# jackroos/VL-BERT

Measured on AMD Instinct MI355X. Metric: samples/sec VL-BERT-base pretrain (seq 64+36 regions) at 1/2/4/8 MI355X, higher is better.
Workload: dtype bf16; 1 GPU; VL-BERT-base 12-layer pretrain step (fwd+bwd+clip+AdamW), 64 text + 36 regions, precomputed 2048-d region features, dropout on; global_batch=256, per_gpu_batch=256, per_gpu_caption_samples=256, per_gpu_text_only_samples=0, module=ResNetVLBERTForPretraining, seq_len=101, parallelism=dp1, hipgraph=False, arch=gfx950:sramecc+:xnack-, cus=256, forced_exchange=False, ranks=1

## Files before the change

### vl-bert_amd/csrc/attention.hip

```cpp
#include "vlb_common.h"

#define ATT_SP_MAX 256
#define ATT_D 64
#define ATT_THREADS 512

typedef __attribute__((ext_vector_type(4))) short s16x4;
typedef __attribute__((ext_vector_type(8))) short s16x8;

__device__ __forceinline__ int rho(int s) { return (s & ~31) | (((s >> 2) & 1) << 4) | (((s >> 3) & 3) << 2) | (s & 3); }
__device__ __forceinline__ int rm_addr(int row, int chunk) { return row * 128 + ((chunk ^ ((row >> 1) & 7)) << 4); }
__device__ __forceinline__ bf16x8 lds_frag(const char* base, int addr) { return *(const bf16x8*)(base + addr); }

__device__ __forceinline__ bf16x8 frag_perm(const char* img, int blk, int half, int c, int chunk) {
  return lds_frag(img, rm_addr(32 * blk + 16 * half + c, chunk));
}
__device__ __forceinline__ bf16x8 frag_nat(const char* img, int s0, int c, int chunk) {
  return lds_frag(img, rm_addr(rho(s0 + c), chunk));
}
__device__ __forceinline__ bf16x8 frag_tr(const char* img, int blk, int d0, int lane) {
  const int L = lane & 15, g = lane >> 4;
  const int b = d0 * 2 + (L & 3) * 8;
  const int r_lo = 32 * blk + 4 * g + (L >> 2);
  const int r_hi = r_lo + 16;
  const int a_lo = r_lo * 128 + ((((b >> 4) ^ ((r_lo >> 1) & 7)) << 4) | (b & 15));
  const int a_hi = r_hi * 128 + ((((b >> 4) ^ ((r_hi >> 1) & 7)) << 4) | (b & 15));
  const s16x4 lo = __builtin_amdgcn_ds_read_tr16_b64_v4i16((__attribute__((address_space(3))) s16x4*)(img + a_lo));
  const s16x4 hi = __builtin_amdgcn_ds_read_tr16_b64_v4i16((__attribute__((address_space(3))) s16x4*)(img + a_hi));
  const s16x8 v = __builtin_shufflevector(lo, hi, 0, 1, 2, 3, 4, 5, 6, 7);
  return __builtin_bit_cast(bf16x8, v);
}

template <int SP>
struct TileRegs {
  uint4 v[SP * 8 / ATT_THREADS];
};

template <int SP>
__device__ __forceinline__ void tile_load(const bf16_t* __restrict__ g, long ld, int S, int tid, TileRegs<SP>& r) {
#pragma unroll
  for (int it = 0; it < SP * 8 / ATT_THREADS; ++it) {
    const int P = it * ATT_THREADS + tid, s = min(P >> 3, S - 1), ch = P & 7;
    r.v[it] = *(const uint4*)(g + (long)s * ld + ch * 8);
  }
}

template <int SP>
__device__ __forceinline__ void tile_store(const TileRegs<SP>& r, int S, char* img, int tid) {
#pragma unroll
  for (int it = 0; it < SP * 8 / ATT_THREADS; ++it) {
    const int P = it * ATT_THREADS + tid, s = P >> 3, ch = P & 7;
    const bool in = s < S;
    const uint4 v = make_uint4(in ? r.v[it].x : 0u, in ? r.v[it].y : 0u, in ? r.v[it].z : 0u, in ? r.v[it].w : 0u);
    *(uint4*)(img + rm_addr(rho(s), ch)) = v;
  }
}

template <int SP>
__device__ __forceinline__ void rowdot_store(const TileRegs<SP>& a_, const TileRegs<SP>& o_, int S, float* sD, int tid) {
#pragma unroll
  for (int it = 0; it < SP * 8 / ATT_THREADS; ++it) {
    const int P = it * ATT_THREADS + tid, row = P >> 3, ch = P & 7;
    const uint4 a = a_.v[it], o = o_.v[it];
    float d = bflo(a.x) * bflo(o.x) + bfhi(a.x) * bfhi(o.x) + bflo(a.y) * bflo(o.y) + bfhi(a.y) * bfhi(o.y) +
              bflo(a.z) * bflo(o.z) + bfhi(a.z) * bfhi(o.z) + bflo(a.w) * bflo(o.w) + bfhi(a.w) * bfhi(o.w);
    d = row < S ? d : 0.f;
    d += __shfl_xor(d, 1, 64);
    d += __shfl_xor(d, 2, 64);
    d += __shfl_xor(d, 4, 64);
    if (ch == 0) sD[row] = d;
  }
}

__device__ __forceinline__ bf16x8 pack8(const float* v) {
  uint32_t w[4] = {pack2bf(v[0], v[1]), pack2bf(v[2], v[3]), pack2bf(v[4], v[5]), pack2bf(v[6], v[7])};
  return __builtin_bit_cast(bf16x8, *(uint4*)w);
}

__device__ __forceinline__ void drop8(float* v, uint32_t key, uint32_t base, uint32_t thr, float scale) {
  const uint32_t odd = base & 1u, p0 = base >> 1;
  uint32_t h[5];
#pragma unroll
  for (int k = 0; k < 5; ++k) h[k] = vlb_pair_hash(p0 + k, key);
#pragma unroll
  for (int k = 0; k < 4; ++k) {
    const uint32_t w = __builtin_amdgcn_alignbit(h[k + 1], h[k], odd << 4);
    v[2 * k] = ((w & 0xffffu) >= thr) ? v[2 * k] * scale : 0.f;
    v[2 * k + 1] = ((w >> 16) >= thr) ? v[2 * k + 1] * scale : 0.f;
  }
}

struct AttnParams {
  const bf16_t* qkv;
  const float* mask;
  bf16_t* ctx;
  float* lse;
  const bf16_t* dctx;
  bf16_t* dqkv;
  int B, S, H, nh;
  float scale;
  uint32_t drop_thr; float drop_scale; const uint32_t* seed; uint32_t tag;
};

template <int NU, int QS>
__global__ __launch_bounds__(ATT_THREADS, NU <= 4 ? 4 : 2) void attn_fwd_kernel(const AttnParams p) {
  constexpr int ATT_SP = 32 * NU, TILE_BYTES = ATT_SP * ATT_D * 2;
  extern __shared__ __attribute__((aligned(16))) char smem[];
  char* sK = smem;
  char* sV = smem + TILE_BYTES;
  float* sMB = (float*)(smem + 2 * TILE_BYTES);

  const int tid = threadIdx.x, lane = tid & 63, wave = tid >> 6;
  const int c = lane & 15, g = lane >> 4;
  const int b = blockIdx.x / p.nh, h = blockIdx.x % p.nh;
  const int S = p.S;
  const long ld = 3L * p.H;
  const bf16_t* qbase = p.qkv + (long)b * S * ld + h * ATT_D;
  TileRegs<ATT_SP> rk, rv;
  tile_load<ATT_SP>(qbase + p.H, ld, S, tid, rk);
  tile_load<ATT_SP>(qbase + 2 * p.H, ld, S, tid, rv);
  bf16x8 qf[2];
  auto load_q = [&](int q0) {
    const int q = min(q0 + c, S - 1);
#pragma unroll
    for (int ds = 0; ds < 2; ++ds) qf[ds] = *(const bf16x8*)(qbase + (long)q * ld + ds * 32 + g * 8);
  };
  load_q(wave * 16);
  const float mrow = p.mask[b * S + min(tid, S - 1)];
  const uint32_t seed = (p.drop_thr && p.seed) ? *p.seed : 0u;
  tile_store<ATT_SP>(rk, S, sK, tid);
  tile_store<ATT_SP>(rv, S, sV, tid);
  if (tid < ATT_SP) sMB[tid] = (tid < S) ? (1.0f - mrow) * -10000.0f : -INFINITY;
  __syncthreads();
  const uint32_t key = vlb_rng_key(seed, p.tag);
  const int U = (S + 31) >> 5;

#pragma unroll 1
  for (int qs = 0; qs < QS; ++qs) {
  const int q0 = (wave + 8 * qs) * 16;
  if (q0 >= S) break;
  if (qs > 0) load_q(q0);

  f32x4 sc[NU][2];
#pragma unroll
  for (int u = 0; u < NU; ++u)
#pragma unroll
    for (int hf = 0; hf < 2; ++hf) {
      sc[u][hf] = (f32x4){0.f, 0.f, 0.f, 0.f};
      if (u < U) {
#pragma unroll
        for (int ds = 0; ds < 2; ++ds)
          sc[u][hf] = VLB_MFMA_16x16x32(frag_perm(sK, u, hf, c, ds * 4 + g), qf[ds], sc[u][hf], 0, 0, 0);
      }
    }

  float mx = -INFINITY;
#pragma unroll
  for (int u = 0; u < NU; ++u)
#pragma unroll
    for (int hf = 0; hf < 2; ++hf)
#pragma unroll
      for (int r = 0; r < 4; ++r) {
        const float v = (u < U) ? sc[u][hf][r] * p.scale + sMB[32 * u + 8 * g + 4 * hf + r] : -INFINITY;
        sc[u][hf][r] = v;
        mx = fmaxf(mx, v);
      }
  mx = fmaxf(mx, __shfl_xor(mx, 16, 64));
  mx = fmaxf(mx, __shfl_xor(mx, 32, 64));
  float sum = 0.f;
#pragma unroll
  for (int u = 0; u < NU; ++u)
#pragma unroll
    for (int hf = 0; hf < 2; ++hf)
#pragma unroll
      for (int r = 0; r < 4; ++r) {
        const float e = __expf(sc[u][hf][r] - mx);
        sc[u][hf][r] = e;
        sum += e;
      }
  sum += __shfl_xor(sum, 16, 64);
  sum += __shfl_xor(sum, 32, 64);
  const float inv = 1.0f / sum;
  const int q = q0 + c;
  if (g == 0 && q < S) p.lse[((long)b * p.nh + h) * S + q] = mx + __logf(sum);

  const uint32_t qrow = ((uint32_t)(b * p.nh + h) * (uint32_t)S + (uint32_t)min(q, S - 1)) * (uint32_t)S;
  bf16x8 pf[NU];
#pragma unroll
  for (int u = 0; u < NU; ++u) {
    float v[8];
#pragma unroll
    for (int hf = 0; hf < 2; ++hf)
#pragma unroll
      for (int r = 0; r < 4; ++r) v[4 * hf + r] = sc[u][hf][r] * inv;
    if (p.drop_thr) drop8(v, key, qrow + 32u * u + 8u * g, p.drop_thr, p.drop_scale);
    pf[u] = pack8(v);
  }

  bf16_t* orow = p.ctx + ((long)b * S + min(q, S - 1)) * p.H + h * ATT_D + 4 * g;
#pragma unroll
  for (int dt = 0; dt < 4; ++dt) {
    f32x4 o = {0.f, 0.f, 0.f, 0.f};
#pragma unroll
    for (int u = 0; u < NU; ++u)
      if (u < U) o = VLB_MFMA_16x16x32(frag_tr(sV, u, dt * 16, lane), pf[u], o, 0, 0, 0);
    if (q < S) *(uint2*)(orow + dt * 16) = make_uint2(pack2bf(o[0], o[1]), pack2bf(o[2], o[3]));
  }
  }
}

template <int NU, int QS>
__global__ __launch_bounds__(ATT_THREADS, NU <= 4 ? 4 : 2) void attn_bwd_kernel(const AttnParams p) {
  constexpr int ATT_SP = 32 * NU, TILE_BYTES = ATT_SP * ATT_D * 2;
  extern __shared__ __attribute__((aligned(16))) char smem[];
  char* sQ = smem;
  char* sK = smem + 1 * TILE_BYTES;
  char* sV = smem + 2 * TILE_BYTES;
  char* sdO = smem + 3 * TILE_BYTES;
  float* sMB = (float*)(smem + 4 * TILE_BYTES);
  float* sLSE = sMB + ATT_SP;
  float* sD = sLSE + ATT_SP;

  const int tid = threadIdx.x, lane = tid & 63, wave = tid >> 6;
  const int c = lane & 15, g = lane >> 4;
  const int b = blockIdx.x / p.nh, h = blockIdx.x % p.nh;
  const int S = p.S;
  const long ld = 3L * p.H;
  const bf16_t* qbase = p.qkv + (long)b * S * ld + h * ATT_D;
  const bf16_t* dobase = p.dctx + (long)b * S * p.H + h * ATT_D;
  const bf16_t* obase = p.ctx + (long)b * S * p.H + h * ATT_D;
  TileRegs<ATT_SP> rq, rk, rv, rdo, ro;
  tile_load<ATT_SP>(qbase, ld, S, tid, rq);
  tile_load<ATT_SP>(qbase + p.H, ld, S, tid, rk);
  tile_load<ATT_SP>(qbase + 2 * p.H, ld, S, tid, rv);
  tile_load<ATT_SP>(dobase, p.H, S, tid, rdo);
  tile_load<ATT_SP>(obase, p.H, S, tid, ro);
  const float mrow = p.mask[b * S + min(tid, S - 1)];
  const float lrow = p.lse[((long)b * p.nh + h) * S + min(tid, S - 1)];
  const uint32_t seed = (p.drop_thr && p.seed) ? *p.seed : 0u;
  tile_store<ATT_SP>(rq, S, sQ, tid);
  tile_store<ATT_SP>(rk, S, sK, tid);
  tile_store<ATT_SP>(rv, S, sV, tid);
  tile_store<ATT_SP>(rdo, S, sdO, tid);
  rowdot_store<ATT_SP>(rdo, ro, S, sD, tid);
  if (tid < ATT_SP) {
    sMB[tid] = (tid < S) ? (1.0f - mrow) * -10000.0f : -INFINITY;
    sLSE[tid] = (tid < S) ? lrow : 0.f;
  }
  __syncthreads();

  const uint32_t key = vlb_rng_key(seed, p.tag);
  const uint32_t bh = (uint32_t)(b * p.nh + h);
  const int U = (S + 31) >> 5;
#pragma unroll 1
  for (int qs = 0; qs < QS; ++qs) {
  const int w16 = (wave + 8 * qs) * 16;
  if (w16 >= S) break;
  const int pos = w16 + c;
  const bool pos_ok = pos < S;

  {
    bf16x8 kf[2], vf[2];
#pragma unroll
    for (int ds = 0; ds < 2; ++ds) {
      kf[ds] = frag_nat(sK, w16, c, ds * 4 + g);
      vf[ds] = frag_nat(sV, w16, c, ds * 4 + g);
    }
    f32x4 dv[4], dk[4];
#pragma unroll
    for (int dt = 0; dt < 4; ++dt) dv[dt] = dk[dt] = (f32x4){0.f, 0.f, 0.f, 0.f};
    const float mb = sMB[pos];
    const uint32_t kcol = (uint32_t)min(pos, S - 1);
#pragma unroll (NU <= 4 ? NU : 1)
    for (int v = 0; v < NU; ++v) {
      if (v < U) {
        float pv[8], dsv[8];
#pragma unroll
        for (int hf = 0; hf < 2; ++hf) {
          f32x4 s = {0.f, 0.f, 0.f, 0.f}, dp = {0.f, 0.f, 0.f, 0.f};
#pragma unroll
          for (int ds = 0; ds < 2; ++ds) {
            s = VLB_MFMA_16x16x32(frag_perm(sQ, v, hf, c, ds * 4 + g), kf[ds], s, 0, 0, 0);
            dp = VLB_MFMA_16x16x32(frag_perm(sdO, v, hf, c, ds * 4 + g), vf[ds], dp, 0, 0, 0);
          }
#pragma unroll
          for (int r = 0; r < 4; ++r) {
            const int q = 32 * v + 8 * g + 4 * hf + r;
            const float pr = __expf(s[r] * p.scale + mb - sLSE[q]);
            float keepf = 1.f;
            if (p.drop_thr) {
              const uint32_t idx = (bh * (uint32_t)S + (uint32_t)min(q, S - 1)) * (uint32_t)S + kcol;
              const uint32_t hsh = vlb_pair_hash(idx >> 1, key);
              keepf = (((idx & 1u) ? (hsh >> 16) : (hsh & 0xffffu)) >= p.drop_thr) ? p.drop_scale : 0.f;
            }
            pv[4 * hf + r] = pr * keepf;
            dsv[4 * hf + r] = pr * (dp[r] * keepf - sD[q]);
          }
        }
        const bf16x8 pd = pack8(pv), dsf = pack8(dsv);
#pragma unroll
        for (int dt = 0; dt < 4; ++dt) {
          dv[dt] = VLB_MFMA_16x16x32(frag_tr(sdO, v, dt * 16, lane), pd, dv[dt], 0, 0, 0);
          dk[dt] = VLB_MFMA_16x16x32(frag_tr(sQ, v, dt * 16, lane), dsf, dk[dt], 0, 0, 0);
        }
      }
    }
    if (pos_ok) {
      bf16_t* orow = p.dqkv + ((long)b * S + pos) * ld + h * ATT_D + 4 * g;
#pragma unroll
      for (int dt = 0; dt < 4; ++dt) {
        *(uint2*)(orow + p.H + dt * 16) = make_uint2(pack2bf(dk[dt][0] * p.scale, dk[dt][1] * p.scale),
                                                     pack2bf(dk[dt][2] * p.scale, dk[dt][3] * p.scale));
        *(uint2*)(orow + 2 * p.H + dt * 16) = make_uint2(pack2bf(dv[dt][0], dv[dt][1]), pack2bf(dv[dt][2], dv[dt][3]));
      }
    }
  }

  {
    bf16x8 qf[2], dof[2];
#pragma unroll
    for (int ds = 0; ds < 2; ++ds) {
      qf[ds] = frag_nat(sQ, w16, c, ds * 4 + g);
      dof[ds] = frag_nat(sdO, w16, c, ds * 4 + g);
    }
    f32x4 dq[4];
#pragma unroll
    for (int dt = 0; dt < 4; ++dt) dq[dt] = (f32x4){0.f, 0.f, 0.f, 0.f};
    const float lse = sLSE[pos], dd = sD[pos];
    const uint32_t qrow = (bh * (uint32_t)S + (uint32_t)min(pos, S - 1)) * (uint32_t)S;
#pragma unroll (NU <= 4 ? NU : 1)
    for (int u = 0; u < NU; ++u) {
      if (u < U) {
        float pr[8], dpv[8];
#pragma unroll
        for (int hf = 0; hf < 2; ++hf) {
          f32x4 s = {0.f, 0.f, 0.f, 0.f}, dp = {0.f, 0.f, 0.f, 0.f};
#pragma unroll
          for (int ds = 0; ds < 2; ++ds) {
            s = VLB_MFMA_16x16x32(frag_perm(sK, u, hf, c, ds * 4 + g), qf[ds], s, 0, 0, 0);
            dp = VLB_MFMA_16x16x32(frag_perm(sV, u, hf, c, ds * 4 + g), dof[ds], dp, 0, 0, 0);
          }
#pragma unroll
          for (int r = 0; r < 4; ++r) {
            pr[4 * hf + r] = __expf(s[r] * p.scale + sMB[32 * u + 8 * g + 4 * hf + r] - lse);
            dpv[4 * hf + r] = dp[r];
          }
        }
        if (p.drop_thr) drop8(dpv, key, qrow + 32u * u + 8u * g, p.drop_thr, p.drop_scale);
        float dsv[8];
#pragma unroll
        for (int j = 0; j < 8; ++j) dsv[j] = pr[j] * (dpv[j] - dd);
        const bf16x8 dsf = pack8(dsv);
#pragma unroll
        for (int dt = 0; dt < 4; ++dt)
          dq[dt] = VLB_MFMA_16x16x32(frag_tr(sK, u, dt * 16, lane), dsf, dq[dt], 0, 0, 0);
      }
    }
    if (pos_ok) {
      bf16_t* orow = p.dqkv + ((long)b * S + pos) * ld + h * ATT_D + 4 * g;
#pragma unroll
      for (int dt = 0; dt < 4; ++dt)
        *(uint2*)(orow + dt * 16) = make_uint2(pack2bf(dq[dt][0] * p.scale, dq[dt][1] * p.scale),
                                               pack2bf(dq[dt][2] * p.scale, dq[dt][3] * p.scale));
    }
  }
  }
}

__device__ __forceinline__ int pt_addr(int row, int chunk16) { return row * 256 + ((chunk16 ^ (row & 15)) << 4); }

__device__ __forceinline__ bf16x8 frag_pt(const char* img, int v, int key0, int lane) {
  const int L = lane & 15, g = lane >> 4;
  const int r_lo = 32 * v + 8 * g + (L >> 2), r_hi = r_lo + 4;
  const int cb = key0 * 2 + (L & 3) * 8;
  const int a_lo = pt_addr(r_lo, cb >> 4) | (cb & 15), a_hi = pt_addr(r_hi, cb >> 4) | (cb & 15);
  const s16x4 lo = __builtin_amdgcn_ds_read_tr16_b64_v4i16((__attribute__((address_space(3))) s16x4*)(img + a_lo));
  const s16x4 hi = __builtin_amdgcn_ds_read_tr16_b64_v4i16((__attribute__((address_space(3))) s16x4*)(img + a_hi));
  const s16x8 w = __builtin_shufflevector(lo, hi, 0, 1, 2, 3, 4, 5, 6, 7);
  return __builtin_bit_cast(bf16x8, w);
}

__global__ __launch_bounds__(ATT_THREADS, 4) void attn_bwd2_kernel(const AttnParams p) {
  constexpr int NU = 4, ATT_SP = 128, TILE_BYTES = ATT_SP * ATT_D * 2;
  extern __shared__ __attribute__((aligned(16))) char smem[];
  char* sQ = smem;
  char* sK = smem + 1 * TILE_BYTES;
  char* sV = smem + 2 * TILE_BYTES;
  char* sdO = smem + 3 * TILE_BYTES;
  char* sT = sK;
  float* sMB = (float*)(smem + 4 * TILE_BYTES);
  float* sLSE = sMB + ATT_SP;
  float* sD = sLSE + ATT_SP;

  const int tid = threadIdx.x, lane = tid & 63, wave = tid >> 6;
  const int c = lane & 15, g = lane >> 4;
  const int b = blockIdx.x / p.nh, h = blockIdx.x % p.nh;
  const int S = p.S;
  const long ld = 3L * p.H;
  const bf16_t* qbase = p.qkv + (long)b * S * ld + h * ATT_D;
  const bf16_t* dobase = p.dctx + (long)b * S * p.H + h * ATT_D;
  const bf16_t* obase = p.ctx + (long)b * S * p.H + h * ATT_D;
  TileRegs<ATT_SP> rq, rk, rv, rdo, ro;
  tile_load<ATT_SP>(qbase, ld, S, tid, rq);
  tile_load<ATT_SP>(qbase + p.H, ld, S, tid, rk);
  tile_load<ATT_SP>(qbase + 2 * p.H, ld, S, tid, rv);
  tile_load<ATT_SP>(dobase, p.H, S, tid, rdo);
  tile_load<ATT_SP>(obase, p.H, S, tid, ro);
  const float mrow = p.mask[b * S + min(tid, S - 1)];
  const float lrow = p.lse[((long)b * p.nh + h) * S + min(tid, S - 1)];
  const uint32_t seed = (p.drop_thr && p.seed) ? *p.seed : 0u;
  tile_store<ATT_SP>(rq, S, sQ, tid);
  tile_store<ATT_SP>(rk, S, sK, tid);
  tile_store<ATT_SP>(rv, S, sV, tid);
  tile_store<ATT_SP>(rdo, S, sdO, tid);
  rowdot_store<ATT_SP>(rdo, ro, S, sD, tid);
  if (tid < ATT_SP) {
    sMB[tid] = (tid < S) ? (1.0f - mrow) * -10000.0f : -INFINITY;
    sLSE[tid] = (tid < S) ? lrow : 0.f;
  }
  __syncthreads();

  const uint32_t key = vlb_rng_key(seed, p.tag);
  const uint32_t bh = (uint32_t)(b * p.nh + h);
  const int U = (S + 31) >> 5;
  const int w16 = wave * 16;
  const int pos = w16 + c;
  const bool pos_ok = pos < S;
  const bool active = w16 < 32 * U;

  bf16x8 pd[NU], dsf[NU];
#pragma unroll
  for (int u = 0; u < NU; ++u) pd[u] = dsf[u] = (bf16x8){0, 0, 0, 0, 0, 0, 0, 0};
  if (w16 < S) {
    bf16x8 qf[2], dof[2];
#pragma unroll
    for (int ds = 0; ds < 2; ++ds) {
      qf[ds] = frag_nat(sQ, w16, c, ds * 4 + g);
      dof[ds] = frag_nat(sdO, w16, c, ds * 4 + g);
    }
    f32x4 dq[4];
#pragma unroll
    for (int dt = 0; dt < 4; ++dt) dq[dt] = (f32x4){0.f, 0.f, 0.f, 0.f};
    const float lse = sLSE[pos], dd = sD[pos];
    const float rowf = pos_ok ? 1.f : 0.f;
    const uint32_t qrow = (bh * (uint32_t)S + (uint32_t)min(pos, S - 1)) * (uint32_t)S;
#pragma unroll
    for (int u = 0; u < NU; ++u) {
      if (u < U) {
        float pr[8], dpv[8], kv[8];
#pragma unroll
        for (int hf = 0; hf < 2; ++hf) {
          f32x4 sc = {0.f, 0.f, 0.f, 0.f}, dp = {0.f, 0.f, 0.f, 0.f};
#pragma unroll
          for (int ds = 0; ds < 2; ++ds) {
            sc = VLB_MFMA_16x16x32(frag_perm(sK, u, hf, c, ds * 4 + g), qf[ds], sc, 0, 0, 0);
            dp = VLB_MFMA_16x16x32(frag_perm(sV, u, hf, c, ds * 4 + g), dof[ds], dp, 0, 0, 0);
          }
#pragma unroll
          for (int r = 0; r < 4; ++r) {
            pr[4 * hf + r] = __expf(sc[r] * p.scale + sMB[32 * u + 8 * g + 4 * hf + r] - lse) * rowf;
            dpv[4 * hf + r] = dp[r];
            kv[4 * hf + r] = 1.f;
          }
        }
        if (p.drop_thr) drop8(kv, key, qrow + 32u * u + 8u * g, p.drop_thr, p.drop_scale);
        float pdv[8], dsv[8];
#pragma unroll
        for (int j = 0; j < 8; ++j) {
          pdv[j] = pr[j] * kv[j];
          dsv[j] = pr[j] * (dpv[j] * kv[j] - dd);
        }
        pd[u] = pack8(pdv);
        dsf[u] = pack8(dsv);
#pragma unroll
        for (int dt = 0; dt < 4; ++dt)
          dq[dt] = VLB_MFMA_16x16x32(frag_tr(sK, u, dt * 16, lane), dsf[u], dq[dt], 0, 0, 0);
      }
    }
    if (pos_ok) {
      bf16_t* orow = p.dqkv + ((long)b * S + pos) * ld + h * ATT_D + 4 * g;
#pragma unroll
      for (int dt = 0; dt < 4; ++dt)
        *(uint2*)(orow + dt * 16) = make_uint2(pack2bf(dq[dt][0] * p.scale, dq[dt][1] * p.scale),
                                               pack2bf(dq[dt][2] * p.scale, dq[dt][3] * p.scale));
    }
  }
  __syncthreads();

  f32x4 dv[4], dk[4];
#pragma unroll
  for (int dt = 0; dt < 4; ++dt) dv[dt] = dk[dt] = (f32x4){0.f, 0.f, 0.f, 0.f};
  if (active) {
#pragma unroll
    for (int u = 0; u < NU; ++u)
      if (u < U) *(bf16x8*)(sT + pt_addr(w16 + c, 4 * u + g)) = pd[u];
  }
  __syncthreads();
  if (w16 < S) {
#pragma unroll
    for (int v = 0; v < NU; ++v) {
      if (v < U) {
        const bf16x8 pt = frag_pt(sT, v, w16, lane);
#pragma unroll
        for (int dt = 0; dt < 4; ++dt)
          dv[dt] = VLB_MFMA_16x16x32(frag_tr(sdO, v, dt * 16, lane), pt, dv[dt], 0, 0, 0);
      }
    }
  }
  __syncthreads();
  if (active) {
#pragma unroll
    for (int u = 0; u < NU; ++u)
      if (u < U) *(bf16x8*)(sT + pt_addr(w16 + c, 4 * u + g)) = dsf[u];
  }
  __syncthreads();
  if (w16 < S) {
#pragma unroll
    for (int v = 0; v < NU; ++v) {
      if (v < U) {
        const bf16x8 st = frag_pt(sT, v, w16, lane);
#pragma unroll
        for (int dt = 0; dt < 4; ++dt)
          dk[dt] = VLB_MFMA_16x16x32(frag_tr(sQ, v, dt * 16, lane), st, dk[dt], 0, 0, 0);
      }
    }
    if (pos_ok) {
      bf16_t* orow = p.dqkv + ((long)b * S + pos) * ld + h * ATT_D + 4 * g;
#pragma unroll
      for (int dt = 0; dt < 4; ++dt) {
        *(uint2*)(orow + p.H + dt * 16) = make_uint2(pack2bf(dk[dt][0] * p.scale, dk[dt][1] * p.scale),
                                                     pack2bf(dk[dt][2] * p.scale, dk[dt][3] * p.scale));
        *(uint2*)(orow + 2 * p.H + dt * 16) = make_uint2(pack2bf(dv[dt][0], dv[dt][1]), pack2bf(dv[dt][2], dv[dt][3]));
      }
    }
  }
}

static int check_attn(const char* name, int B, int S, int H, int nh) {
  VLB_CHECK_ARG(B > 0 && S > 0 && S <= ATT_SP_MAX, "%s: S=%d unsupported (1..%d)", name, S, ATT_SP_MAX);
  VLB_CHECK_ARG(nh > 0 && H == nh * ATT_D, "%s: head dim must be 64 (H=%d, heads=%d)", name, H, nh);
  VLB_CHECK_ARG((long)B * nh * S * S < (1L << 32), "%s: dropout index overflow", name);
  return VLB_OK;
}

extern "C" int vlb_attention_fwd(const void* qkv, const float* mask, void* ctx, float* lse, int B, int S, int H, int nh,
                                 float drop_p, const uint32_t* seed, uint32_t tag, hipStream_t stream) {
  int rc = check_attn("vlb_attention_fwd", B, S, H, nh);
  if (rc) return rc;
  VLB_CHECK_ARG(qkv && mask && ctx && lse, "vlb_attention_fwd: null argument");
  VLB_CHECK_ARG(!(drop_p > 0.f) || seed, "vlb_attention_fwd: dropout needs a device seed pointer");
  AttnParams p;
  p.qkv = (const bf16_t*)qkv; p.mask = mask; p.ctx = (bf16_t*)ctx; p.lse = lse; p.dctx = nullptr; p.dqkv = nullptr;
  p.B = B; p.S = S; p.H = H; p.nh = nh; p.scale = 0.125f;
  p.drop_thr = vlb_drop_thr(drop_p); p.drop_scale = vlb_drop_scale(p.drop_thr); p.seed = seed; p.tag = tag;
  if (S <= 128) {
    const int smem = 2 * (128 * ATT_D * 2) + 128 * 4;
    hipLaunchKernelGGL((attn_fwd_kernel<4, 1>), dim3(B * nh), dim3(ATT_THREADS), smem, stream, p);
  } else {
    const int smem = 2 * (256 * ATT_D * 2) + 256 * 4;
    static bool attr_set = false;
    if (!attr_set) {
      (void)hipFuncSetAttribute((const void*)attn_fwd_kernel<8, 2>, hipFuncAttributeMaxDynamicSharedMemorySize, smem);
      attr_set = true;
    }
    hipLaunchKernelGGL((attn_fwd_kernel<8, 2>), dim3(B * nh), dim3(ATT_THREADS), smem, stream, p);
  }
  VLB_CHECK_LAUNCH("vlb_attention_fwd");
  return VLB_OK;
}

extern "C" int vlb_attention_bwd(const void* qkv, const float* mask, const void* ctx, const float* lse, const void* dctx,
                                 void* dqkv, int B, int S, int H, int nh, float drop_p, const uint32_t* seed, uint32_t tag,
                                 hipStream_t stream) {
  int rc = check_attn("vlb_attention_bwd", B, S, H, nh);
  if (rc) return rc;
  VLB_CHECK_ARG(qkv && mask && ctx && lse && dctx && dqkv, "vlb_attention_bwd: null argument");
  VLB_CHECK_ARG(!(drop_p > 0.f) || seed, "vlb_attention_bwd: dropout needs a device seed pointer");
  AttnParams p;
  p.qkv = (const bf16_t*)qkv; p.mask = mask; p.ctx = (bf16_t*)ctx; p.lse = (float*)lse; p.dctx = (const bf16_t*)dctx;
  p.dqkv = (bf16_t*)dqkv;
  p.B = B; p.S = S; p.H = H; p.nh = nh; p.scale = 0.125f;
  p.drop_thr = vlb_drop_thr(drop_p); p.drop_scale = vlb_drop_scale(p.drop_thr); p.seed = seed; p.tag = tag;
  static bool attr_set = false;
  if (!attr_set) {
    (void)hipFuncSetAttribute((const void*)attn_bwd_kernel<4, 1>, hipFuncAttributeMaxDynamicSharedMemorySize, 4 * (128 * ATT_D * 2) + 3 * 128 * 4);
    (void)hipFuncSetAttribute((const void*)attn_bwd2_kernel, hipFuncAttributeMaxDynamicSharedMemorySize, 4 * (128 * ATT_D * 2) + 3 * 128 * 4);
    (void)hipFuncSetAttribute((const void*)attn_bwd_kernel<8, 2>, hipFuncAttributeMaxDynamicSharedMemorySize, 4 * (256 * ATT_D * 2) + 3 * 256 * 4);
    attr_set = true;
  }
  static int bwd2 = -1;
  if (bwd2 < 0) {
    const char* v = getenv("VLB_ATTN_BWD2");
    bwd2 = v ? atoi(v) : 1;
  }
  if (S <= 128 && bwd2)
    hipLaunchKernelGGL(attn_bwd2_kernel, dim3(B * nh), dim3(ATT_THREADS), 4 * (128 * ATT_D * 2) + 3 * 128 * 4, stream, p);
  else if (S <= 128)
    hipLaunchKernelGGL((attn_bwd_kernel<4, 1>), dim3(B * nh), dim3(ATT_THREADS), 4 * (128 * ATT_D * 2) + 3 * 128 * 4, stream, p);
  else
    hipLaunchKernelGGL((attn_bwd_kernel<8, 2>), dim3(B * nh), dim3(ATT_THREADS), 4 * (256 * ATT_D * 2) + 3 * 256 * 4, stream, p);
  VLB_CHECK_LAUNCH("vlb_attention_bwd");
  return VLB_OK;
}
```

Baseline: 13700 samples/s.

## Add 16-key tail blocks in fused attention backward and retune LDS swizzles

```diff
diff --git a/vl-bert_amd/csrc/attention.hip b/vl-bert_amd/csrc/attention.hip
--- a/vl-bert_amd/csrc/attention.hip
+++ b/vl-bert_amd/csrc/attention.hip
@@ -1,3 +1,5 @@
+#include <type_traits>
+
 #include "vlb_common.h"
 
 #define ATT_SP_MAX 256
@@ -8,24 +10,27 @@
 typedef __attribute__((ext_vector_type(8))) short s16x8;
 
 __device__ __forceinline__ int rho(int s) { return (s & ~31) | (((s >> 2) & 1) << 4) | (((s >> 3) & 3) << 2) | (s & 3); }
-__device__ __forceinline__ int rm_addr(int row, int chunk) { return row * 128 + ((chunk ^ ((row >> 1) & 7)) << 4); }
+__device__ __forceinline__ int rho_t(int s, int t0) { return s >= t0 ? s : rho(s); }
+__device__ __forceinline__ int rm_addr(int row, int chunk) { return row * 128 + ((chunk ^ (row & 6)) << 4); }
 __device__ __forceinline__ bf16x8 lds_frag(const char* base, int addr) { return *(const bf16x8*)(base + addr); }
 
 __device__ __forceinline__ bf16x8 frag_perm(const char* img, int blk, int half, int c, int chunk) {
   return lds_frag(img, rm_addr(32 * blk + 16 * half + c, chunk));
 }
-__device__ __forceinline__ bf16x8 frag_nat(const char* img, int s0, int c, int chunk) {
-  return lds_frag(img, rm_addr(rho(s0 + c), chunk));
-}
+__device__ __forceinline__ bf16x8 frag_nat(const char* img, int s0, int c, int chunk, int t0 = ATT_SP_MAX) {
+  return lds_frag(img, rm_addr(rho_t(s0 + c, t0), chunk));
+}
+__device__ __forceinline__ s16x4 lds_tr(const char* img, int addr) {
+  return __builtin_amdgcn_ds_read_tr16_b64_v4i16((__attribute__((address_space(3))) s16x4*)(img + addr));
+}
+template <bool TAIL = false>
 __device__ __forceinline__ bf16x8 frag_tr(const char* img, int blk, int d0, int lane) {
   const int L = lane & 15, g = lane >> 4;
   const int b = d0 * 2 + (L & 3) * 8;
   const int r_lo = 32 * blk + 4 * g + (L >> 2);
   const int r_hi = r_lo + 16;
-  const int a_lo = r_lo * 128 + ((((b >> 4) ^ ((r_lo >> 1) & 7)) << 4) | (b & 15));
-  const int a_hi = r_hi * 128 + ((((b >> 4) ^ ((r_hi >> 1) & 7)) << 4) | (b & 15));
-  const s16x4 lo = __builtin_amdgcn_ds_read_tr16_b64_v4i16((__attribute__((address_space(3))) s16x4*)(img + a_lo));
-  const s16x4 hi = __builtin_amdgcn_ds_read_tr16_b64_v4i16((__attribute__((address_space(3))) s16x4*)(img + a_hi));
+  const s16x4 lo = lds_tr(img, rm_addr(r_lo, b >> 4) | (b & 15));
+  const s16x4 hi = TAIL ? (s16x4){0, 0, 0, 0} : lds_tr(img, rm_addr(r_hi, b >> 4) | (b & 15));
   const s16x8 v = __builtin_shufflevector(lo, hi, 0, 1, 2, 3, 4, 5, 6, 7);
   return __builtin_bit_cast(bf16x8, v);
 }
@@ -45,13 +50,13 @@
 }
 
 template <int SP>
-__device__ __forceinline__ void tile_store(const TileRegs<SP>& r, int S, char* img, int tid) {
+__device__ __forceinline__ void tile_store(const TileRegs<SP>& r, int S, char* img, int tid, int t0 = ATT_SP_MAX) {
 #pragma unroll
   for (int it = 0; it < SP * 8 / ATT_THREADS; ++it) {
     const int P = it * ATT_THREADS + tid, s = P >> 3, ch = P & 7;
     const bool in = s < S;
     const uint4 v = make_uint4(in ? r.v[it].x : 0u, in ? r.v[it].y : 0u, in ? r.v[it].z : 0u, in ? r.v[it].w : 0u);
-    *(uint4*)(img + rm_addr(rho(s), ch)) = v;
+    *(uint4*)(img + rm_addr(rho_t(s, t0), ch)) = v;
   }
 }
 
@@ -76,17 +81,31 @@
   return __builtin_bit_cast(bf16x8, *(uint4*)w);
 }
 
-__device__ __forceinline__ void drop8(float* v, uint32_t key, uint32_t base, uint32_t thr, float scale) {
+template <int N>
+__device__ __forceinline__ void dropn(float* v, uint32_t key, uint32_t base, uint32_t thr, float scale) {
   const uint32_t odd = base & 1u, p0 = base >> 1;
-  uint32_t h[5];
-#pragma unroll
-  for (int k = 0; k < 5; ++k) h[k] = vlb_pair_hash(p0 + k, key);
-#pragma unroll
-  for (int k = 0; k < 4; ++k) {
+  uint32_t h[N / 2 + 1];
+#pragma unroll
+  for (int k = 0; k < N / 2 + 1; ++k) h[k] = vlb_pair_hash(p0 + k, key);
+#pragma unroll
+  for (int k = 0; k < N / 2; ++k) {
     const uint32_t w = __builtin_amdgcn_alignbit(h[k + 1], h[k], odd << 4);
     v[2 * k] = ((w & 0xffffu) >= thr) ? v[2 * k] * scale : 0.f;
     v[2 * k + 1] = ((w >> 16) >= thr) ? v[2 * k + 1] * scale : 0.f;
   }
+}
+
+struct KeyBlocks {
+  int uf, t0;
+  bool tail;
+};
+template <bool TAILS>
+__device__ __forceinline__ KeyBlocks key_blocks(int S) {
+  KeyBlocks kb;
+  kb.uf = TAILS ? (S + 15) >> 5 : (S + 31) >> 5;
+  kb.tail = TAILS && 32 * kb.uf < S;
+  kb.t0 = kb.tail ? 32 * kb.uf : ATT_SP_MAX;
+  return kb;
 }
 
 struct AttnParams {
@@ -192,7 +211,7 @@
     for (int hf = 0; hf < 2; ++hf)
 #pragma unroll
       for (int r = 0; r < 4; ++r) v[4 * hf + r] = sc[u][hf][r] * inv;
-    if (p.drop_thr) drop8(v, key, qrow + 32u * u + 8u * g, p.drop_thr, p.drop_scale);
+    if (p.drop_thr) dropn<8>(v, key, qrow + 32u * u + 8u * g, p.drop_thr, p.drop_scale);
     pf[u] = pack8(v);
   }
 
@@ -345,7 +364,7 @@
             dpv[4 * hf + r] = dp[r];
           }
         }
-        if (p.drop_thr) drop8(dpv, key, qrow + 32u * u + 8u * g, p.drop_thr, p.drop_scale);
+        if (p.drop_thr) dropn<8>(dpv, key, qrow + 32u * u + 8u * g, p.drop_thr, p.drop_scale);
         float dsv[8];
 #pragma unroll
         for (int j = 0; j < 8; ++j) dsv[j] = pr[j] * (dpv[j] - dd);
@@ -366,15 +385,18 @@
   }
 }
 
-__device__ __forceinline__ int pt_addr(int row, int chunk16) { return row * 256 + ((chunk16 ^ (row & 15)) << 4); }
-
+__device__ __forceinline__ int pt_addr(int row, int chunk16) {
+  const int sw = ((row >> 2) & 1) | ((row & 3) << 1) | ((((row >> 2) ^ (row >> 3)) & 1) << 3);
+  return row * 256 + ((chunk16 ^ sw) << 4);
+}
+
+template <bool TAIL = false>
 __device__ __forceinline__ bf16x8 frag_pt(const char* img, int v, int key0, int lane) {
   const int L = lane & 15, g = lane >> 4;
-  const int r_lo = 32 * v + 8 * g + (L >> 2), r_hi = r_lo + 4;
+  const int r_lo = 32 * v + (TAIL ? 4 : 8) * g + (L >> 2), r_hi = r_lo + 4;
   const int cb = key0 * 2 + (L & 3) * 8;
-  const int a_lo = pt_addr(r_lo, cb >> 4) | (cb & 15), a_hi = pt_addr(r_hi, cb >> 4) | (cb & 15);
-  const s16x4 lo = __builtin_amdgcn_ds_read_tr16_b64_v4i16((__attribute__((address_space(3))) s16x4*)(img + a_lo));
-  const s16x4 hi = __builtin_amdgcn_ds_read_tr16_b64_v4i16((__attribute__((address_space(3))) s16x4*)(img + a_hi));
+  const s16x4 lo = lds_tr(img, pt_addr(r_lo, cb >> 4) | (cb & 15));
+  const s16x4 hi = TAIL ? (s16x4){0, 0, 0, 0} : lds_tr(img, pt_addr(r_hi, cb >> 4) | (cb & 15));
   const s16x8 w = __builtin_shufflevector(lo, hi, 0, 1, 2, 3, 4, 5, 6, 7);
   return __builtin_bit_cast(bf16x8, w);
 }
@@ -408,10 +430,12 @@
   const float mrow = p.mask[b * S + min(tid, S - 1)];
   const float lrow = p.lse[((long)b * p.nh + h) * S + min(tid, S - 1)];
   const uint32_t seed = (p.drop_thr && p.seed) ? *p.seed : 0u;
-  tile_store<ATT_SP>(rq, S, sQ, tid);
-  tile_store<ATT_SP>(rk, S, sK, tid);
-  tile_store<ATT_SP>(rv, S, sV, tid);
-  tile_store<ATT_SP>(rdo, S, sdO, tid);
+  const KeyBlocks kb = key_blocks<true>(S);
+  const int UF = kb.uf;
+  tile_store<ATT_SP>(rq, S, sQ, tid, kb.t0);
+  tile_store<ATT_SP>(rk, S, sK, tid, kb.t0);
+  tile_store<ATT_SP>(rv, S, sV, tid, kb.t0);
+  tile_store<ATT_SP>(rdo, S, sdO, tid, kb.t0);
   rowdot_store<ATT_SP>(rdo, ro, S, sD, tid);
   if (tid < ATT_SP) {
     sMB[tid] = (tid < S) ? (1.0f - mrow) * -10000.0f : -INFINITY;
@@ -421,11 +445,10 @@
 
   const uint32_t key = vlb_rng_key(seed, p.tag);
   const uint32_t bh = (uint32_t)(b * p.nh + h);
-  const int U = (S + 31) >> 5;
   const int w16 = wave * 16;
   const int pos = w16 + c;
   const bool pos_ok = pos < S;
-  const bool active = w16 < 32 * U;
+  const bool active = w16 < 32 * UF + (kb.tail ? 16 : 0);
 
   bf16x8 pd[NU], dsf[NU];
 #pragma unroll
@@ -434,8 +457,8 @@
     bf16x8 qf[2], dof[2];
 #pragma unroll
     for (int ds = 0; ds < 2; ++ds) {
-      qf[ds] = frag_nat(sQ, w16, c, ds * 4 + g);
-      dof[ds] = frag_nat(sdO, w16, c, ds * 4 + g);
+      qf[ds] = frag_nat(sQ, w16, c, ds * 4 + g, kb.t0);
+      dof[ds] = frag_nat(sdO, w16, c, ds * 4 + g, kb.t0);
     }
     f32x4 dq[4];
 #pragma unroll
@@ -443,38 +466,50 @@
     const float lse = sLSE[pos], dd = sD[pos];
     const float rowf = pos_ok ? 1.f : 0.f;
     const uint32_t qrow = (bh * (uint32_t)S + (uint32_t)min(pos, S - 1)) * (uint32_t)S;
+    auto block = [&](const int u, auto tail_c) __attribute__((always_inline)) {
+      constexpr bool TAIL = decltype(tail_c)::value;
+      float pr[8], dpv[8], kv[8];
+#pragma unroll
+      for (int hf = 0; hf < 2; ++hf) {
+        if (TAIL && hf == 1) {
+#pragma unroll
+          for (int r = 0; r < 4; ++r) pr[4 + r] = dpv[4 + r] = 0.f, kv[4 + r] = 1.f;
+          continue;
+        }
+        f32x4 sc = {0.f, 0.f, 0.f, 0.f}, dp = {0.f, 0.f, 0.f, 0.f};
+#pragma unroll
+        for (int ds = 0; ds < 2; ++ds) {
+          sc = VLB_MFMA_16x16x32(frag_perm(sK, u, hf, c, ds * 4 + g), qf[ds], sc, 0, 0, 0);
+          dp = VLB_MFMA_16x16x32(frag_perm(sV, u, hf, c, ds * 4 + g), dof[ds], dp, 0, 0, 0);
+        }
+#pragma unroll
+        for (int r = 0; r < 4; ++r) {
+          const int kk = TAIL ? 32 * u + 4 * g + r : 32 * u + 8 * g + 4 * hf + r;
+          pr[4 * hf + r] = __expf(sc[r] * p.scale + sMB[kk] - lse) * rowf;
+          dpv[4 * hf + r] = dp[r];
+          kv[4 * hf + r] = 1.f;
+        }
+      }
+      if (p.drop_thr) {
+        if (TAIL) dropn<4>(kv, key, qrow + 32u * u + 4u * g, p.drop_thr, p.drop_scale);
+        else dropn<8>(kv, key, qrow + 32u * u + 8u * g, p.drop_thr, p.drop_scale);
+      }
+      float pdv[8], dsv[8];
+#pragma unroll
+      for (int j = 0; j < 8; ++j) {
+        pdv[j] = pr[j] * kv[j];
+        dsv[j] = pr[j] * (dpv[j] * kv[j] - dd);
+      }
+      pd[u] = pack8(pdv);
+      dsf[u] = pack8(dsv);
+#pragma unroll
+      for (int dt = 0; dt < 4; ++dt)
+        dq[dt] = VLB_MFMA_16x16x32(frag_tr<TAIL>(sK, u, dt * 16, lane), dsf[u], dq[dt], 0, 0, 0);
+    };
 #pragma unroll
     for (int u = 0; u < NU; ++u) {
-      if (u < U) {
-        float pr[8], dpv[8], kv[8];
-#pragma unroll
-        for (int hf = 0; hf < 2; ++hf) {
-          f32x4 sc = {0.f, 0.f, 0.f, 0.f}, dp = {0.f, 0.f, 0.f, 0.f};
-#pragma unroll
-          for (int ds = 0; ds < 2; ++ds) {
-            sc = VLB_MFMA_16x16x32(frag_perm(sK, u, hf, c, ds * 4 + g), qf[ds], sc, 0, 0, 0);
-            dp = VLB_MFMA_16x16x32(frag_perm(sV, u, hf, c, ds * 4 + g), dof[ds], dp, 0, 0, 0);
-          }
-#pragma unroll
-          for (int r = 0; r < 4; ++r) {
-            pr[4 * hf + r] = __expf(sc[r] * p.scale + sMB[32 * u + 8 * g + 4 * hf + r] - lse) * rowf;
-            dpv[4 * hf + r] = dp[r];
-            kv[4 * hf + r] = 1.f;
-          }
-        }
-        if (p.drop_thr) drop8(kv, key, qrow + 32u * u + 8u * g, p.drop_thr, p.drop_scale);
-        float pdv[8], dsv[8];
-#pragma unroll
-        for (int j = 0; j < 8; ++j) {
-          pdv[j] = pr[j] * kv[j];
-          dsv[j] = pr[j] * (dpv[j] * kv[j] - dd);
-        }
-        pd[u] = pack8(pdv);
-        dsf[u] = pack8(dsv);
-#pragma unroll
-        for (int dt = 0; dt < 4; ++dt)
-          dq[dt] = VLB_MFMA_16x16x32(frag_tr(sK, u, dt * 16, lane), dsf[u], dq[dt], 0, 0, 0);
-      }
+      if (u < UF) block(u, std::false_type{});
+      else if (kb.tail && u == UF) block(u, std::true_type{});
     }
     if (pos_ok) {
       bf16_t* orow = p.dqkv + ((long)b * S + pos) * ld + h * ATT_D + 4 * g;
@@ -491,36 +526,56 @@
   for (int dt = 0; dt < 4; ++dt) dv[dt] = dk[dt] = (f32x4){0.f, 0.f, 0.f, 0.f};
   if (active) {
 #pragma unroll
-    for (int u = 0; u < NU; ++u)
-      if (u < U) *(bf16x8*)(sT + pt_addr(w16 + c, 4 * u + g)) = pd[u];
+    for (int u = 0; u < NU; ++u) {
+      if (u < UF) *(bf16x8*)(sT + pt_addr(w16 + c, 4 * u + g)) = pd[u];
+      else if (kb.tail && u == UF) {
+        const uint4 w = __builtin_bit_cast(uint4, pd[u]);
+        *(uint2*)(sT + (pt_addr(w16 + c, 4 * u + (g >> 1)) | (8 * (g & 1)))) = make_uint2(w.x, w.y);
+      }
+    }
   }
   __syncthreads();
   if (w16 < S) {
 #pragma unroll
     for (int v = 0; v < NU; ++v) {
-      if (v < U) {
+      if (v < UF) {
         const bf16x8 pt = frag_pt(sT, v, w16, lane);
 #pragma unroll
         for (int dt = 0; dt < 4; ++dt)
           dv[dt] = VLB_MFMA_16x16x32(frag_tr(sdO, v, dt * 16, lane), pt, dv[dt], 0, 0, 0);
+      } else if (kb.tail && v == UF) {
+        const bf16x8 pt = frag_pt<true>(sT, v, w16, lane);
+#pragma unroll
+        for (int dt = 0; dt < 4; ++dt)
+          dv[dt] = VLB_MFMA_16x16x32(frag_tr<true>(sdO, v, dt * 16, lane), pt, dv[dt], 0, 0, 0);
       }
     }
   }
   __syncthreads();
   if (active) {
 #pragma unroll
-    for (int u = 0; u < NU; ++u)
-      if (u < U) *(bf16x8*)(sT + pt_addr(w16 + c, 4 * u + g)) = dsf[u];
+    for (int u = 0; u < NU; ++u) {
+      if (u < UF) *(bf16x8*)(sT + pt_addr(w16 + c, 4 * u + g)) = dsf[u];
+      else if (kb.tail && u == UF) {
+        const uint4 w = __builtin_bit_cast(uint4, dsf[u]);
+        *(uint2*)(sT + (pt_addr(w16 + c, 4 * u + (g >> 1)) | (8 * (g & 1)))) = make_uint2(w.x, w.y);
+      }
+    }
   }
   __syncthreads();
   if (w16 < S) {
 #pragma unroll
     for (int v = 0; v < NU; ++v) {
-      if (v < U) {
+      if (v < UF) {
         const bf16x8 st = frag_pt(sT, v, w16, lane);
 #pragma unroll
         for (int dt = 0; dt < 4; ++dt)
           dk[dt] = VLB_MFMA_16x16x32(frag_tr(sQ, v, dt * 16, lane), st, dk[dt], 0, 0, 0);
+      } else if (kb.tail && v == UF) {
+        const bf16x8 st = frag_pt<true>(sT, v, w16, lane);
+#pragma unroll
+        for (int dt = 0; dt < 4; ++dt)
+          dk[dt] = VLB_MFMA_16x16x32(frag_tr<true>(sQ, v, dt * 16, lane), st, dk[dt], 0, 0, 0);
       }
     }
     if (pos_ok) {
```

Result: no change. 13650 samples/s (median of 2 runs) (-0.4%).
